# orneryd/NornicDB

Measured on AMD Instinct MI355X. Metric: kNN QPS @ recall>=0.95 on 100Mx1024 bge-m3 vectors + embed docs/sec, higher is better.
Workload: dtype bf16; 1 GPU; model=bge-m3 (XLM-R-large shape: 24L/1024h/16heads, random init), global_batch=256, seq_len=256, corpus_vectors=100000000, dim=1024, k=10

## Files before the change

nornicdb_amd/csrc/knn_mfma.hip:

```cpp

#include <torch/extension.h>
#include <ATen/hip/HIPContext.h>
#include "common.h"
#include "allow_mask.h"

typedef __bf16 bf16x8 __attribute__((ext_vector_type(8)));

#define G_AS __attribute__((address_space(1)))
#define L_AS __attribute__((address_space(3)))

#ifndef KNN_BM
#define KNN_BM 96
#endif
#define BM KNN_BM
#define BN 256
#define BK 64
#define NTHREADS 256
#define KCAND 10
#define MW (BM / 16)

__device__ __forceinline__ int swz(int b) {
  return (b & ~127) | ((b & 127) ^ (((b >> 7) & 7) << 4));
}

template <bool FILTERED>
__global__ __launch_bounds__(NTHREADS, 3) void k_knn_mfma(
    const unsigned short* __restrict__ db, const unsigned short* __restrict__ qs,
    long long n_panels,
    int d,
    long long row_base, float* __restrict__ cand_score,
    int* __restrict__ cand_idx, const unsigned int* __restrict__ allow) {
  static_assert(!FILTERED || BM % 32 == 0,
                "filtered kNN needs whole mask words per panel");
  __shared__ __align__(16) char smem[BM * BK * 2 + BN * BK * 2];
  unsigned short* sA = (unsigned short*)smem;
  unsigned short* sB = (unsigned short*)(smem + BM * BK * 2);
  float* sT = (float*)smem;

  const int tid = threadIdx.x;
  const int lane = tid & (WAVE - 1);
  const int wc = tid / WAVE;

  float tv[KCAND];
  int ti[KCAND];
#pragma unroll
  for (int i = 0; i < KCAND; ++i) { tv[i] = -1e30f; ti[i] = -1; }

  const long long d2 = (long long)d * 2;

  for (long long panel = blockIdx.x; panel < n_panels; panel += gridDim.x) {
    const long long prow = panel * BM;

    unsigned int aw[(BM + 31) / 32];
    if constexpr (FILTERED) {
      unsigned int any = 0;
#pragma unroll
      for (int h = 0; h < BM / 32; ++h) {
        aw[h] = allow[(prow >> 5) + h];
        any |= aw[h];
      }
      if (any == 0) continue;
    }

    float4v acc[MW][4];
#pragma unroll
    for (int m = 0; m < MW; ++m)
#pragma unroll
      for (int nn = 0; nn < 4; ++nn) acc[m][nn] = {0.f, 0.f, 0.f, 0.f};

    for (int kt = 0; kt < d; kt += BK) {
#pragma unroll
      for (int it = 0; it < BM / 32; ++it) {
        int chunk = wc * (BM / 32) + it;
        int x = chunk * 1024 + lane * 16;
        int p = swz(x);
        const G_AS unsigned int* gp = (const G_AS unsigned int*)(
            (const char*)db + (prow + (p >> 7)) * d2 + (long long)kt * 2 +
            (p & 127));
        L_AS unsigned int* lp = (L_AS unsigned int*)((char*)sA + chunk * 1024);
        __builtin_amdgcn_global_load_lds(gp, lp, 16, 0, 0);
      }
#pragma unroll
      for (int it = 0; it < 8; ++it) {
        int chunk = wc * 8 + it;
        int x = chunk * 1024 + lane * 16;
        int p = swz(x);
        const G_AS unsigned int* gp = (const G_AS unsigned int*)(
            (const char*)qs + (long long)(p >> 7) * d2 + (long long)kt * 2 +
            (p & 127));
        L_AS unsigned int* lp = (L_AS unsigned int*)((char*)sB + chunk * 1024);
        __builtin_amdgcn_global_load_lds(gp, lp, 16, 0, 0);
      }
      __syncthreads();

#pragma unroll
      for (int ks = 0; ks < 2; ++ks) {
        const int kb = (ks * 32 + (lane >> 4) * 8) * 2;
        bf16x8 bfr[4];
#pragma unroll
        for (int nn = 0; nn < 4; ++nn) {
          int c = wc * 64 + nn * 16 + (lane & 15);
          bfr[nn] = (bf16x8)(*reinterpret_cast<const short8v*>(
              (const char*)sB + swz(c * 128 + kb)));
        }
#pragma unroll
        for (int m = 0; m < MW; ++m) {
          int r = m * 16 + (lane & 15);
          bf16x8 af = (bf16x8)(*reinterpret_cast<const short8v*>(
              (const char*)sA + swz(r * 128 + kb)));
#pragma unroll
          for (int nn = 0; nn < 4; ++nn)
            acc[m][nn] = __builtin_amdgcn_mfma_f32_16x16x32_bf16(
                af, bfr[nn], acc[m][nn], 0, 0, 0);
        }
      }
      __syncthreads();
    }

#pragma unroll
    for (int h = 0; h < BM / 32; ++h) {
#pragma unroll
      for (int mi = 0; mi < 2; ++mi) {
        int m = h * 2 + mi;
#pragma unroll
        for (int nn = 0; nn < 4; ++nn) {
          int col = wc * 64 + nn * 16 + (lane & 15);
          int srow = mi * 16 + (lane >> 4) * 4;
          *reinterpret_cast<float4v*>(sT + col * 36 + srow) = acc[m][nn];
        }
      }
      __syncthreads();
      const long long grow0 = prow + (long long)h * 32;
#pragma unroll
      for (int j = 0; j < 32; j += 4) {
        float4v v = *reinterpret_cast<const float4v*>(sT + tid * 36 + j);
#pragma unroll
        for (int e = 0; e < 4; ++e) {
          float s = v[e];
          bool ok = s > tv[KCAND - 1];
          if constexpr (FILTERED) ok = ok && ((aw[h] >> (j + e)) & 1u);
          if (ok) {
            float cs = s;
            int ci = (int)(grow0 + j + e);
#pragma unroll
            for (int i = 0; i < KCAND; ++i) {
              bool ins = cs > tv[i];
              float ts = tv[i]; int tj = ti[i];
              tv[i] = ins ? cs : tv[i];
              ti[i] = ins ? ci : ti[i];
              cs = ins ? ts : cs; ci = ins ? tj : ci;
            }
          }
        }
      }
      __syncthreads();
    }
  }

  long long slot = (long long)blockIdx.x * BN + tid;
#pragma unroll
  for (int i = 0; i < KCAND; ++i) {
    cand_score[slot * KCAND + i] = tv[i];
    cand_idx[slot * KCAND + i] = ti[i];
  }
}

template <int K>
__global__ void k_topk_merge_i32(const float* __restrict__ cand_score,
                                 const int* __restrict__ cand_idx,
                                 long long w, int q_stride, int k_out,
                                 long long row_base,
                                 float* __restrict__ out_score,
                                 long long* __restrict__ out_idx) {
  const int q = blockIdx.x;
  const long long total = w * K;
  const int lane = threadIdx.x & (WAVE - 1);
  const int wid = threadIdx.x / WAVE;
  __shared__ unsigned long long s_best[8];

  float tv[K];
  int ti[K];
#pragma unroll
  for (int i = 0; i < K; ++i) { tv[i] = -1e30f; ti[i] = -1; }
  for (long long j = threadIdx.x; j < total; j += blockDim.x) {
    long long src = ((j / K) * q_stride + q) * K + (j % K);
    float s = cand_score[src];
    if (s > tv[K - 1]) {
      int ci = cand_idx[src];
      float cs = s;
#pragma unroll
      for (int i = 0; i < K; ++i) {
        bool ins = cs > tv[i];
        float ts = tv[i]; int tj = ti[i];
        tv[i] = ins ? cs : tv[i];
        ti[i] = ins ? ci : ti[i];
        cs = ins ? ts : cs; ci = ins ? tj : ci;
      }
    }
  }

  unsigned int mono;
  int head = 0;
  for (int r = 0; r < k_out; ++r) {
    float hv = -1e30f;
#pragma unroll
    for (int i = 0; i < K; ++i)
      if (i == head) hv = tv[i];
    if (head >= K) hv = -1e30f;
    {
      unsigned int u = __float_as_uint(hv);
      mono = (u & 0x80000000u) ? ~u : (u | 0x80000000u);
    }
    unsigned long long packed =
        ((unsigned long long)mono << 32) | (unsigned int)threadIdx.x;
#pragma unroll
    for (int off = 32; off > 0; off >>= 1) {
      unsigned long long o = __shfl_xor(packed, off, WAVE);
      if (o > packed) packed = o;
    }
    if (lane == 0) s_best[wid] = packed;
    __syncthreads();
    if (threadIdx.x == 0) {
      unsigned long long b = s_best[0];
      for (int i = 1; i < (int)(blockDim.x / WAVE); ++i)
        if (s_best[i] > b) b = s_best[i];
      s_best[0] = b;
    }
    __syncthreads();
    int winner = (int)(s_best[0] & 0xffffffffu);
    if (threadIdx.x == winner) {
      float wv = -1e30f; int wi = -1;
#pragma unroll
      for (int i = 0; i < K; ++i)
        if (i == head) { wv = tv[i]; wi = ti[i]; }
      out_score[(long long)q * k_out + r] = wv;
      out_idx[(long long)q * k_out + r] = (wi < 0) ? -1 : row_base + wi;
      head++;
    }
    __syncthreads();
  }
}

std::tuple<at::Tensor, at::Tensor> knn_mfma(at::Tensor db, at::Tensor q,
                                            long long row_base, int k_out,
                                            c10::optional<at::Tensor> allow) {
  TORCH_CHECK(db.is_cuda() && db.dim() == 2 && db.is_contiguous() &&
                  db.scalar_type() == at::kBFloat16,
              "knn_mfma: db must be contiguous 2D bf16 CUDA");
  TORCH_CHECK(q.is_cuda() && q.dim() == 2 && q.is_contiguous() &&
                  q.scalar_type() == at::kBFloat16,
              "knn_mfma: q must be contiguous 2D bf16 CUDA");
  long long n = db.size(0);
  int d = (int)db.size(1);
  TORCH_CHECK(q.size(0) == BN, "knn_mfma: q must be padded to ", BN, " rows");
  TORCH_CHECK(q.size(1) == d, "dim mismatch");
  TORCH_CHECK(d % BK == 0, "knn_mfma needs D % 64 == 0");
  TORCH_CHECK(n % BM == 0, "knn_mfma needs N % ", BM, " == 0 (python pads/tails)");
  TORCH_CHECK(n < (1LL << 31), "shard too large for int32 local rows");
  TORCH_CHECK(k_out >= 1 && k_out <= KCAND);
  const unsigned int* allow_p = nullptr;
  if (allow.has_value()) allow_p = check_allow_mask(*allow, db, n, "knn_mfma");

  long long n_panels = n / BM;
  int max_grid = 7680;
  if (const char* g = getenv("NORNICDB_KNN_GRID")) max_grid = atoi(g);
  int grid = (int)std::min<long long>(n_panels, max_grid);
  auto stream = at::hip::getCurrentHIPStream().stream();

  auto opts_f = db.options().dtype(at::kFloat);
  auto opts_i32 = db.options().dtype(at::kInt);
  auto opts_i64 = db.options().dtype(at::kLong);
  at::Tensor cand_s = at::empty({grid, BN, KCAND}, opts_f);
  at::Tensor cand_i = at::empty({grid, BN, KCAND}, opts_i32);

  if (allow_p == nullptr) {
    hipLaunchKernelGGL(k_knn_mfma<false>, dim3(grid), dim3(NTHREADS), 0,
                       stream, (const unsigned short*)db.data_ptr(),
                       (const unsigned short*)q.data_ptr(), n_panels, d,
                       row_base, cand_s.data_ptr<float>(),
                       cand_i.data_ptr<int>(), allow_p);
  } else {
#if KNN_BM % 32 == 0
    hipLaunchKernelGGL(k_knn_mfma<true>, dim3(grid), dim3(NTHREADS), 0,
                       stream, (const unsigned short*)db.data_ptr(),
                       (const unsigned short*)q.data_ptr(), n_panels, d,
                       row_base, cand_s.data_ptr<float>(),
                       cand_i.data_ptr<int>(), allow_p);
#else
    TORCH_CHECK(false, "knn_mfma: filtered search needs KNN_BM % 32 == 0");
#endif
  }
  HIP_CHECK_LAST();

  at::Tensor out_s = at::empty({BN, k_out}, opts_f);
  at::Tensor out_i = at::empty({BN, k_out}, opts_i64);
  hipLaunchKernelGGL((k_topk_merge_i32<KCAND>), dim3(BN), dim3(256), 0, stream,
                     cand_s.data_ptr<float>(), cand_i.data_ptr<int>(), grid,
                     BN, k_out, row_base, out_s.data_ptr<float>(),
                     reinterpret_cast<long long*>(out_i.data_ptr<int64_t>()));
  HIP_CHECK_LAST();
  return {out_s, out_i};
}

long long knn_bm_value() { return BM; }
```

Before: 2215 queries/s (each query embedded by bge-m3 then searched over full corpus).

## Software-pipeline kNN MFMA kernel with multi-buffered LDS and cross-panel prefetch

Rewrites the brute-force kNN MFMA kernel's main loop. It now uses a double-buffered query tile and a triple-buffered corpus tile with BK=32, and prefetches the next panel's first stages while the current panel finishes. It also interleaves LDS fragment reads with MFMAs through hand-placed waitcnt, sched_barrier and setprio, moves the epilogue to 16-row slices through a spare LDS buffer, and raises BM to 160 with a smaller grid. This targets the load-sync-compute stalls of the old single-buffered loop, at the cost of occupancy (2 WGs/CU), a more register-heavy tile, and inline asm that relies on exact waitcnt accounting.

```diff
diff --git a/nornicdb_amd/csrc/knn_mfma.hip b/nornicdb_amd/csrc/knn_mfma.hip
--- a/nornicdb_amd/csrc/knn_mfma.hip
+++ b/nornicdb_amd/csrc/knn_mfma.hip
@@ -1,6 +1,7 @@
 
 #include <torch/extension.h>
 #include <ATen/hip/HIPContext.h>
+#include <type_traits>
 #include "common.h"
 #include "allow_mask.h"
 
@@ -10,138 +11,236 @@
 #define L_AS __attribute__((address_space(3)))
 
 #ifndef KNN_BM
-#define KNN_BM 96
+#define KNN_BM 160
 #endif
 #define BM KNN_BM
 #define BN 256
-#define BK 64
+#define BK 32
 #define NTHREADS 256
 #define KCAND 10
 #define MW (BM / 16)
 
+#define SB_BYTES (BN * BK * 2)
+#define SA_BYTES (BM * BK * 2)
+#define SMEM_BYTES (2 * SB_BYTES + 3 * SA_BYTES)
+
+#define A_PIECES (BM / 16)
+#define A_FULL (A_PIECES / 4)
+#define A_HALF (A_PIECES % 4 == 2 ? 1 : 0)
+#define NA (A_FULL + A_HALF)
+#define NB (BN / 16 / 4)
+static_assert(A_PIECES % 4 == 0 || A_PIECES % 4 == 2,
+              "corpus stage must split evenly over 4 waves");
+#define KNN_WGS (BM <= 96 ? 3 : 2)
+static_assert(SMEM_BYTES * KNN_WGS <= 160 * 1024, "LDS budget per CU");
+
+namespace knn_mfma_detail {
+
 __device__ __forceinline__ int swz(int b) {
-  return (b & ~127) | ((b & 127) ^ (((b >> 7) & 7) << 4));
+  return b ^ (((b >> 8) & 1) << 5);
+}
+
+template <int I, int N, class F>
+__device__ __forceinline__ void static_for(F&& f) {
+  if constexpr (I < N) {
+    f(std::integral_constant<int, I>{});
+    static_for<I + 1, N>(f);
+  }
+}
+
+template <int OFF, class T>
+__device__ __forceinline__ void ds_read128(T& dst, unsigned addr) {
+  asm volatile("ds_read_b128 %0, %1 offset:%2" : "=v"(dst) : "v"(addr), "n"(OFF));
+}
+template <int OFF>
+__device__ __forceinline__ void ds_write128(unsigned addr, float4v v) {
+  asm volatile("ds_write_b128 %0, %1 offset:%2" ::"v"(addr), "v"(v), "n"(OFF)
+               : "memory");
+}
+template <int N>
+__device__ __forceinline__ void wait_lgkm() {
+  asm volatile("s_waitcnt lgkmcnt(%0)" ::"n"(N) : "memory");
+  __builtin_amdgcn_sched_barrier(0);
+}
+template <int N>
+__device__ __forceinline__ void wait_vm() {
+  asm volatile("s_waitcnt vmcnt(%0)" ::"n"(N) : "memory");
+}
+
+__device__ __forceinline__ void glds(const char* gbase, unsigned voff,
+                                     char* lds) {
+  __builtin_amdgcn_global_load_lds(
+      (const G_AS unsigned int*)(gbase + voff), (L_AS unsigned int*)lds, 16, 0,
+      0);
+}
+
 }
 
 template <bool FILTERED>
-__global__ __launch_bounds__(NTHREADS, 3) void k_knn_mfma(
+__global__ __launch_bounds__(NTHREADS, KNN_WGS) void k_knn_mfma(
     const unsigned short* __restrict__ db, const unsigned short* __restrict__ qs,
     long long n_panels,
     int d,
     long long row_base, float* __restrict__ cand_score,
     int* __restrict__ cand_idx, const unsigned int* __restrict__ allow) {
+  using namespace knn_mfma_detail;
   static_assert(!FILTERED || BM % 32 == 0,
                 "filtered kNN needs whole mask words per panel");
-  __shared__ __align__(16) char smem[BM * BK * 2 + BN * BK * 2];
-  unsigned short* sA = (unsigned short*)smem;
-  unsigned short* sB = (unsigned short*)(smem + BM * BK * 2);
-  float* sT = (float*)smem;
+  __shared__ __align__(16) char smem[SMEM_BYTES];
 
   const int tid = threadIdx.x;
   const int lane = tid & (WAVE - 1);
-  const int wc = tid / WAVE;
+  const int wc = __builtin_amdgcn_readfirstlane(tid / WAVE);
 
   float tv[KCAND];
   int ti[KCAND];
 #pragma unroll
   for (int i = 0; i < KCAND; ++i) { tv[i] = -1e30f; ti[i] = -1; }
 
-  const long long d2 = (long long)d * 2;
-
-  for (long long panel = blockIdx.x; panel < n_panels; panel += gridDim.x) {
-    const long long prow = panel * BM;
-
-    unsigned int aw[(BM + 31) / 32];
+  const int d2 = d * 2;
+  const int nstage = d / BK;
+
+  auto next_live = [&](long long p) -> long long {
     if constexpr (FILTERED) {
-      unsigned int any = 0;
-#pragma unroll
-      for (int h = 0; h < BM / 32; ++h) {
-        aw[h] = allow[(prow >> 5) + h];
-        any |= aw[h];
+      while (p < n_panels) {
+        unsigned int any = 0;
+#pragma unroll
+        for (int h = 0; h < BM / 32; ++h) any |= allow[((p * BM) >> 5) + h];
+        if (any != 0) break;
+        p += gridDim.x;
       }
-      if (any == 0) continue;
-    }
-
-    float4v acc[MW][4];
-#pragma unroll
-    for (int m = 0; m < MW; ++m)
-#pragma unroll
-      for (int nn = 0; nn < 4; ++nn) acc[m][nn] = {0.f, 0.f, 0.f, 0.f};
-
-    for (int kt = 0; kt < d; kt += BK) {
-#pragma unroll
-      for (int it = 0; it < BM / 32; ++it) {
-        int chunk = wc * (BM / 32) + it;
-        int x = chunk * 1024 + lane * 16;
-        int p = swz(x);
-        const G_AS unsigned int* gp = (const G_AS unsigned int*)(
-            (const char*)db + (prow + (p >> 7)) * d2 + (long long)kt * 2 +
-            (p & 127));
-        L_AS unsigned int* lp = (L_AS unsigned int*)((char*)sA + chunk * 1024);
-        __builtin_amdgcn_global_load_lds(gp, lp, 16, 0, 0);
+    }
+    return p;
+  };
+
+  long long panel = next_live(blockIdx.x);
+  if (panel < n_panels) {
+    const unsigned voff =
+        (unsigned)((lane >> 2) * d2 +
+                   (((lane & 3) ^ (((lane >> 4) & 1) << 1)) << 4));
+    const char* qbase = (const char*)qs + (long long)(wc * 64) * d2;
+
+    auto issue_b = [&](int s, int boff) {
+      const char* g = qbase + s * (BK * 2);
+#pragma unroll
+      for (int c = 0; c < NB; ++c)
+        glds(g + (long long)(c * 16) * d2, voff,
+                smem + boff + (wc * NB + c) * 1024);
+    };
+    auto issue_a = [&](long long prow, int s, int aoff) {
+      const char* g = (const char*)db + prow * d2 + s * (BK * 2);
+#pragma unroll
+      for (int c = 0; c < A_FULL; ++c)
+        glds(g + (long long)((wc * A_FULL + c) * 16) * d2, voff,
+                    smem + aoff + (wc * A_FULL + c) * 1024);
+      if constexpr (A_HALF) {
+        if (lane < 32)
+          glds(g + (long long)(4 * A_FULL * 16 + wc * 8) * d2, voff,
+                      smem + aoff + 4 * A_FULL * 1024 + wc * 512);
       }
-#pragma unroll
-      for (int it = 0; it < 8; ++it) {
-        int chunk = wc * 8 + it;
-        int x = chunk * 1024 + lane * 16;
-        int p = swz(x);
-        const G_AS unsigned int* gp = (const G_AS unsigned int*)(
-            (const char*)qs + (long long)(p >> 7) * d2 + (long long)kt * 2 +
-            (p & 127));
-        L_AS unsigned int* lp = (L_AS unsigned int*)((char*)sB + chunk * 1024);
-        __builtin_amdgcn_global_load_lds(gp, lp, 16, 0, 0);
+    };
+
+    const unsigned foff = (unsigned)swz((lane & 15) * 64 + (lane >> 4) * 16);
+    const unsigned lds0 = (unsigned)(unsigned long long)(L_AS char*)smem;
+    const unsigned fb = lds0 + wc * (64 * BK * 2) + foff;
+    const unsigned fa = lds0 + foff;
+    const unsigned ew = lds0 + wc * 4096 + (lane & 15) * 64 +
+                        (((lane >> 4) ^ ((lane >> 2) & 3)) << 4);
+    const unsigned er = tid * 64 + (((tid >> 2) & 3) << 4);
+
+    int b_cur = 0, b_nxt = SB_BYTES;
+    int a_cur = 2 * SB_BYTES, a_nxt = a_cur + SA_BYTES, a_nn = a_nxt + SA_BYTES;
+
+    issue_a(panel * BM, 0, a_cur);
+    issue_b(0, b_cur);
+    issue_a(panel * BM, 1, a_nxt);
+    wait_vm<NA>();
+    __builtin_amdgcn_s_barrier();
+
+    for (;;) {
+      const long long prow = panel * BM;
+      const long long nxt = next_live(panel + gridDim.x);
+      const long long prow_pf = (nxt < n_panels ? nxt : panel) * BM;
+
+      unsigned int aw[(BM + 31) / 32];
+      if constexpr (FILTERED) {
+#pragma unroll
+        for (int h = 0; h < BM / 32; ++h) aw[h] = allow[(prow >> 5) + h];
       }
-      __syncthreads();
-
-#pragma unroll
-      for (int ks = 0; ks < 2; ++ks) {
-        const int kb = (ks * 32 + (lane >> 4) * 8) * 2;
-        bf16x8 bfr[4];
-#pragma unroll
-        for (int nn = 0; nn < 4; ++nn) {
-          int c = wc * 64 + nn * 16 + (lane & 15);
-          bfr[nn] = (bf16x8)(*reinterpret_cast<const short8v*>(
-              (const char*)sB + swz(c * 128 + kb)));
+
+      float4v acc[MW][4];
+#pragma unroll
+      for (int m = 0; m < MW; ++m)
+#pragma unroll
+        for (int nn = 0; nn < 4; ++nn) acc[m][nn] = {0.f, 0.f, 0.f, 0.f};
+
+      for (int s = 0; s < nstage; ++s) {
+        issue_b(s + 1 == nstage ? 0 : s + 1, b_nxt);
+        {
+          const bool wrap = s + 2 >= nstage;
+          issue_a(wrap ? prow_pf : prow, wrap ? s + 2 - nstage : s + 2, a_nn);
         }
-#pragma unroll
-        for (int m = 0; m < MW; ++m) {
-          int r = m * 16 + (lane & 15);
-          bf16x8 af = (bf16x8)(*reinterpret_cast<const short8v*>(
-              (const char*)sA + swz(r * 128 + kb)));
+
+        constexpr int AH = (MW + 1) / 2;
+        bf16x8 bfr[4], afr[AH];
+        const unsigned rb = fb + b_cur, ra = fa + a_cur;
+        static_for<0, 4>([&](auto nn) {
+          ds_read128<decltype(nn)::value * 1024>(bfr[decltype(nn)::value], rb);
+        });
+        static_for<0, AH>([&](auto m) {
+          ds_read128<decltype(m)::value * 1024>(afr[decltype(m)::value], ra);
+        });
+        __builtin_amdgcn_s_setprio(1);
+        static_for<0, MW>([&](auto mc) {
+          constexpr int m = decltype(mc)::value;
+          constexpr int more = m < MW - AH ? m : MW - AH;
+          wait_lgkm<AH - 1 + more - m>();
 #pragma unroll
           for (int nn = 0; nn < 4; ++nn)
             acc[m][nn] = __builtin_amdgcn_mfma_f32_16x16x32_bf16(
-                af, bfr[nn], acc[m][nn], 0, 0, 0);
+                afr[m % AH], bfr[nn], acc[m][nn], 0, 0, 0);
+          if constexpr (m + AH < MW) {
+            __builtin_amdgcn_sched_barrier(0);
+            ds_read128<(m + AH) * 1024>(afr[m % AH], ra);
+          }
+        });
+        __builtin_amdgcn_s_setprio(0);
+
+        wait_vm<NA>();
+        __builtin_amdgcn_s_barrier();
+        __builtin_amdgcn_sched_barrier(0);
+        {
+          int t = b_cur; b_cur = b_nxt; b_nxt = t;
+          t = a_cur; a_cur = a_nxt; a_nxt = a_nn; a_nn = t;
         }
       }
-      __syncthreads();
-    }
-
-#pragma unroll
-    for (int h = 0; h < BM / 32; ++h) {
-#pragma unroll
-      for (int mi = 0; mi < 2; ++mi) {
-        int m = h * 2 + mi;
-#pragma unroll
-        for (int nn = 0; nn < 4; ++nn) {
-          int col = wc * 64 + nn * 16 + (lane & 15);
-          int srow = mi * 16 + (lane >> 4) * 4;
-          *reinterpret_cast<float4v*>(sT + col * 36 + srow) = acc[m][nn];
-        }
-      }
-      __syncthreads();
-      const long long grow0 = prow + (long long)h * 32;
-#pragma unroll
-      for (int j = 0; j < 32; j += 4) {
-        float4v v = *reinterpret_cast<const float4v*>(sT + tid * 36 + j);
-#pragma unroll
-        for (int e = 0; e < 4; ++e) {
-          float s = v[e];
+
+      asm volatile("s_nop 15\n\ts_nop 15" ::: "memory");
+      const unsigned ewb = ew + b_nxt, erb = lds0 + b_nxt;
+      static_for<0, MW>([&](auto mc) {
+        constexpr int m = decltype(mc)::value;
+        static_for<0, 4>([&](auto nn) {
+          ds_write128<decltype(nn)::value * 1024>(ewb,
+                                                  acc[m][decltype(nn)::value]);
+        });
+        wait_lgkm<0>();
+        __builtin_amdgcn_s_barrier();
+        float4v v[4];
+        static_for<0, 4>([&](auto sl) {
+          ds_read128<0>(v[decltype(sl)::value],
+                        erb + (er ^ (unsigned)(decltype(sl)::value << 4)));
+        });
+        wait_lgkm<0>();
+        const long long grow0 = prow + m * 16;
+#pragma unroll
+        for (int j = 0; j < 16; ++j) {
+          float s = v[j >> 2][j & 3];
           bool ok = s > tv[KCAND - 1];
-          if constexpr (FILTERED) ok = ok && ((aw[h] >> (j + e)) & 1u);
+          if constexpr (FILTERED)
+            ok = ok && ((aw[m >> 1] >> ((m & 1) * 16 + j)) & 1u);
           if (ok) {
             float cs = s;
-            int ci = (int)(grow0 + j + e);
+            int ci = (int)(grow0 + j);
 #pragma unroll
             for (int i = 0; i < KCAND; ++i) {
               bool ins = cs > tv[i];
@@ -152,9 +251,14 @@
             }
           }
         }
-      }
-      __syncthreads();
-    }
+        __builtin_amdgcn_s_barrier();
+        __builtin_amdgcn_sched_barrier(0);
+      });
+
+      if (nxt >= n_panels) break;
+      panel = nxt;
+    }
+    wait_vm<0>();
   }
 
   long long slot = (long long)blockIdx.x * BN + tid;
@@ -239,6 +343,17 @@
     }
     __syncthreads();
   }
+}
+
+template <bool FILTERED>
+static void launch_knn_mfma(int grid, hipStream_t stream, const at::Tensor& db,
+                            const at::Tensor& q, long long n_panels, int d,
+                            long long row_base, at::Tensor& cand_s,
+                            at::Tensor& cand_i, const unsigned int* allow_p) {
+  hipLaunchKernelGGL((k_knn_mfma<FILTERED>), dim3(grid), dim3(NTHREADS),
+                     0, stream, (const unsigned short*)db.data_ptr(),
+                     (const unsigned short*)q.data_ptr(), n_panels, d, row_base,
+                     cand_s.data_ptr<float>(), cand_i.data_ptr<int>(), allow_p);
 }
 
 std::tuple<at::Tensor, at::Tensor> knn_mfma(at::Tensor db, at::Tensor q,
@@ -254,7 +369,7 @@
   int d = (int)db.size(1);
   TORCH_CHECK(q.size(0) == BN, "knn_mfma: q must be padded to ", BN, " rows");
   TORCH_CHECK(q.size(1) == d, "dim mismatch");
-  TORCH_CHECK(d % BK == 0, "knn_mfma needs D % 64 == 0");
+  TORCH_CHECK(d % 64 == 0, "knn_mfma needs D % 64 == 0");
   TORCH_CHECK(n % BM == 0, "knn_mfma needs N % ", BM, " == 0 (python pads/tails)");
   TORCH_CHECK(n < (1LL << 31), "shard too large for int32 local rows");
   TORCH_CHECK(k_out >= 1 && k_out <= KCAND);
@@ -262,7 +377,7 @@
   if (allow.has_value()) allow_p = check_allow_mask(*allow, db, n, "knn_mfma");
 
   long long n_panels = n / BM;
-  int max_grid = 7680;
+  int max_grid = 1536;
   if (const char* g = getenv("NORNICDB_KNN_GRID")) max_grid = atoi(g);
   int grid = (int)std::min<long long>(n_panels, max_grid);
   auto stream = at::hip::getCurrentHIPStream().stream();
@@ -274,18 +389,12 @@
   at::Tensor cand_i = at::empty({grid, BN, KCAND}, opts_i32);
 
   if (allow_p == nullptr) {
-    hipLaunchKernelGGL(k_knn_mfma<false>, dim3(grid), dim3(NTHREADS), 0,
-                       stream, (const unsigned short*)db.data_ptr(),
-                       (const unsigned short*)q.data_ptr(), n_panels, d,
-                       row_base, cand_s.data_ptr<float>(),
-                       cand_i.data_ptr<int>(), allow_p);
+    launch_knn_mfma<false>(grid, stream, db, q, n_panels, d, row_base, cand_s,
+                           cand_i, allow_p);
   } else {
 #if KNN_BM % 32 == 0
-    hipLaunchKernelGGL(k_knn_mfma<true>, dim3(grid), dim3(NTHREADS), 0,
-                       stream, (const unsigned short*)db.data_ptr(),
-                       (const unsigned short*)q.data_ptr(), n_panels, d,
-                       row_base, cand_s.data_ptr<float>(),
-                       cand_i.data_ptr<int>(), allow_p);
+    launch_knn_mfma<true>(grid, stream, db, q, n_panels, d, row_base, cand_s,
+                          cand_i, allow_p);
 #else
     TORCH_CHECK(false, "knn_mfma: filtered search needs KNN_BM % 32 == 0");
 #endif
```

New measurement: 2355 queries/s (each query embedded by bge-m3 then searched over full corpus), median of 6. 1.06x the previous value.
